# gk969/stm32-speech-recognition

Measured on AMD Instinct MI355X. Metric: utterances/sec (256-frame, 100 templates), higher is better.
Workload: dtype int32

## Files before the change

profiles/experiments/dtw_stats.py:

```python
import ctypes, json, os, sys
import numpy as np, torch
sys.path.insert(0, os.getcwd())
import bench
from stm32_speech_recognition_amd import Engine, synth
from stm32_speech_recognition_amd import engine as E

which = sys.argv[1] if len(sys.argv) > 1 else "ref"
gain = float(sys.argv[2]) if len(sys.argv) > 2 else 1.0
B = 8192
rate, cfg, Kt, n_words = bench.workload_setup(which, None)
dev = torch.device("cuda", 0)
bank = synth.word_bank(n_words)
eng = Engine(max_frames=bench.MAX_FRAMES, device=0, **cfg)
tm, tfr, rng = bench.make_templates(eng, bank, Kt, n_words, rate, dev, gain)
eng.set_templates_dense(tm, tfr.astype(np.uint32))
pcm = synth.make_utterances(torch.from_numpy(rng.integers(0, n_words, B)), [bench.T] * B, seed=1000, bank=bank,
                            S=synth.buf_len_for(bench.T, rate), device=dev, rate=rate, gain=gain)
out = eng.alloc_outputs(B, dev, mfcc=True, vad=True)
eng.set_pipeline(streams=1)
L = E.load_library()
st = (ctypes.c_ulonglong * 8)()
L.sr_debug_dtw_stats(st, 1)
eng.recognize_dev(pcm, out)
torch.cuda.synchronize()
L.sr_debug_dtw_stats(st, 1)
v = list(st)
sc = out["scores"].cpu().numpy().astype(np.int64)
print(json.dumps({"workload": which, "gain": gain, "wave_steps": v[0], "unsafe": v[1], "short": v[2], "beyond_table": v[3], "lost": v[4],
                  "lane_steps": v[5], "no_adv_y": v[6], "no_adv_x": v[7], "frac_no_adv_y": round(v[6] / v[0], 5),
                  "frac_no_adv_x": round(v[7] / v[0], 5), "frac_unsafe": round(v[1] / v[0], 5), "frac_short": round(v[2] / v[0], 5),
                  "frac_beyond": round(v[3] / v[0], 5), "frac_lost": round(v[4] / v[0], 5),
                  "score_median": float(np.median(sc[sc < 0xFFFFFFFF])), "score_p99": float(np.percentile(sc[sc < 0xFFFFFFFF], 99))}))
```

stm32_speech_recognition_amd/csrc/k_dtw.hip:

```cpp
#include "sr_dtw_dev.h"
#include "sr_dtw_plan.h"

namespace sr {

__device__ uint32_t dtw_pair(const int16_t *in, uint32_t in_n, uint32_t in_rows, const int16_t *mdl, uint32_t mdl_n,
                             uint32_t mdl_rows)
{
    if (in_n > mdl_n * 2 || 2 * in_n < mdl_n) return SR_DIS_ERR;
    const int X1 = (int)(((2 * (int)mdl_n - (int)in_n) / 3) & 0xFFFF);
    const int X2 = (int)(((4 * (int)in_n - 2 * (int)mdl_n) / 3) & 0xFFFF);
    uint32_t px = 0, py = 0;
    Frame12 ci = load_frame(in), cm = load_frame(mdl);
    uint32_t nci = norm2(ci), ncm = norm2(cm);
    uint32_t dis = get_dis_dev(ci, nci, cm, ncm);
    uint32_t step = 1;
    do {
        const uint32_t rx = (px + 1 < in_rows) ? px + 1 : in_rows - 1, ry = (py + 1 < mdl_rows) ? py + 1 : mdl_rows - 1;
        const Frame12 ni = load_frame(in + (size_t)rx * kCoef), nm = load_frame(mdl + (size_t)ry * kCoef);
        const uint32_t nni = norm2(ni), nnm = norm2(nm);
        const int x = (int)px + 1, y = (int)py + 1;
        const uint32_t up = dtw_out(x, y + 1, X1, X2, (int)in_n, (int)mdl_n) ? SR_DIS_ERR : get_dis_dev(nm, nnm, ci, nci);
        const uint32_t right = dtw_out(x + 1, y, X1, X2, (int)in_n, (int)mdl_n) ? SR_DIS_ERR : get_dis_dev(cm, ncm, ni, nni);
        const uint32_t diag =
            dtw_out(x + 1, y + 1, X1, X2, (int)in_n, (int)mdl_n) ? SR_DIS_ERR : get_dis_dev(nm, nnm, ni, nni);
// ... 344 lines not shown
                     "v_pk_mov_b32 %[c3], %[n3], %[n3] op_sel:[0,1]\n\t"
                     "v_pk_mov_b32 %[c4], %[n4], %[n4] op_sel:[0,1]\n\t"
                     "s_mov_b64 exec, %[live]"
                     : [c0] "+v"(c0), [c1] "+v"(c1), [c2] "+v"(c2), [c3] "+v"(c3), [c4] "+v"(c4)
                     : [n0] "v"(n0), [n1] "v"(n1), [n2] "v"(n2), [n3] "v"(n3), [n4] "v"(n4), [k_dg] "s"(k_dg), [k_up] "s"(k_up), [live] "s"(live)
                     : "scc");
        cm.w[0] = c0.x, cm.w[1] = c0.y, cm.w[2] = c1.x, cm.w[3] = c1.y, cm.w[4] = c2.x, cm.w[5] = c2.y, cm.w[6] = c3.x, cm.w[7] = c3.y;
        cm.w[8] = c4.x, cm.w[9] = c4.y;
        u32x4 q0 = {nm.w[0], nm.w[1], nm.w[2], nm.w[3]}, q1 = {nm.w[4], nm.w[5], nm.w[6], nm.w[7]};
        u32x2 q2 = {nm.w[8], nm.w[9]};
        u32x2 a0 = {ci.w[0], ci.w[1]}, a1 = {ci.w[2], ci.w[3]}, a2 = {ci.w[4], ci.w[5]}, a3 = {ci.w[6], ci.w[7]}, b0 = {ni.w[0], ni.w[1]},
              b1 = {ni.w[2], ni.w[3]}, b2 = {ni.w[4], ni.w[5]}, b3 = {ni.w[6], ni.w[7]}, an = {ci.w[8], ni.w[8]};
        asm volatile("s_or_b64 exec, %[k_dg], %[k_up]\n\t" SR_DTW_ADV_Y
                     "global_load_dwordx4 %[q0], %[t_off], %[tbase]\n\t"
                     "global_load_dwordx4 %[q1], %[t_off], %[tbase] offset:16\n\t"
                     "global_load_dwordx2 %[q2], %[t_off], %[tbase] offset:32\n\t" SR_DTW_ADV_X("32")
                     "ds_read_b64 %[a0], %[in_off]\n\t"
                     "ds_read_b64 %[a1], %[in_off] offset:8\n\t"
                     "ds_read_b64 %[a2], %[in_off] offset:16\n\t"
                     "ds_read_b64 %[a3], %[in_off] offset:24\n\t"
                     "ds_read_b64 %[b0], %[in_off] offset:32\n\t"
                     "ds_read_b64 %[b1], %[in_off] offset:40\n\t"
                     "ds_read_b64 %[b2], %[in_off] offset:48\n\t"
                     "ds_read_b64 %[b3], %[in_off] offset:56\n\t" SR_DTW_ADV_END
                     : [q0] "+v"(q0), [q1] "+v"(q1), [q2] "+v"(q2), [a0] "+v"(a0), [a1] "+v"(a1), [a2] "+v"(a2), [a3] "+v"(a3), [b0] "+v"(b0),
                       [b1] "+v"(b1), [b2] "+v"(b2), [b3] "+v"(b3), [an] "+v"(an), SR_DTW_ADV_OPS
                     : SR_DTW_ADV_INS
                     : "memory", "scc");
        nm.w[0] = q0.x, nm.w[1] = q0.y, nm.w[2] = q0.z, nm.w[3] = q0.w, nm.w[4] = q1.x, nm.w[5] = q1.y, nm.w[6] = q1.z, nm.w[7] = q1.w;
        nm.w[8] = q2.x, nm.w[9] = q2.y;
        ci.w[0] = a0.x, ci.w[1] = a0.y, ci.w[2] = a1.x, ci.w[3] = a1.y, ci.w[4] = a2.x, ci.w[5] = a2.y, ci.w[6] = a3.x, ci.w[7] = a3.y;
        ni.w[0] = b0.x, ni.w[1] = b0.y, ni.w[2] = b1.x, ni.w[3] = b1.y, ni.w[4] = b2.x, ni.w[5] = b2.y, ni.w[6] = b3.x, ni.w[7] = b3.y;
        ci.w[8] = an.x, ni.w[8] = an.y;
    }
    static __device__ __forceinline__ void wait_lds(Row &ci, Row &ni)
    {
        u32x2 a0 = {ci.w[0], ci.w[1]}, a1 = {ci.w[2], ci.w[3]}, a2 = {ci.w[4], ci.w[5]}, a3 = {ci.w[6], ci.w[7]}, b0 = {ni.w[0], ni.w[1]},
              b1 = {ni.w[2], ni.w[3]}, b2 = {ni.w[4], ni.w[5]}, b3 = {ni.w[6], ni.w[7]}, an = {ci.w[8], ni.w[8]};
        asm volatile("s_waitcnt lgkmcnt(0)" : "+v"(a0), "+v"(a1), "+v"(a2), "+v"(a3), "+v"(b0), "+v"(b1), "+v"(b2), "+v"(b3), "+v"(an));
        ci.w[0] = a0.x, ci.w[1] = a0.y, ci.w[2] = a1.x, ci.w[3] = a1.y, ci.w[4] = a2.x, ci.w[5] = a2.y, ci.w[6] = a3.x, ci.w[7] = a3.y;
        ni.w[0] = b0.x, ni.w[1] = b0.y, ni.w[2] = b1.x, ni.w[3] = b1.y, ni.w[4] = b2.x, ni.w[5] = b2.y, ni.w[6] = b3.x, ni.w[7] = b3.y;
        ci.w[8] = an.x, ni.w[8] = an.y;
    }
    static __device__ __forceinline__ void wait_tpl(Row &nm)
    {
        u32x4 q0 = {nm.w[0], nm.w[1], nm.w[2], nm.w[3]}, q1 = {nm.w[4], nm.w[5], nm.w[6], nm.w[7]};
        u32x2 q2 = {nm.w[8], nm.w[9]};
        asm volatile("s_waitcnt vmcnt(0)" : "+v"(q0), "+v"(q1), "+v"(q2));
        nm.w[0] = q0.x, nm.w[1] = q0.y, nm.w[2] = q0.z, nm.w[3] = q0.w, nm.w[4] = q1.x, nm.w[5] = q1.y, nm.w[6] = q1.z, nm.w[7] = q1.w;
        nm.w[8] = q2.x, nm.w[9] = q2.y;
    }
};
#ifdef SR_DTW_STATS
__device__ unsigned long long g_dtw_stats[8];
extern "C" void sr_debug_dtw_stats(unsigned long long *out, int reset)
{
    (void)hipDeviceSynchronize();
    (void)hipMemcpyFromSymbol(out, HIP_SYMBOL(g_dtw_stats), sizeof(g_dtw_stats));
    if (reset) {
        unsigned long long z[8] = {0};
        (void)hipMemcpyToSymbol(HIP_SYMBOL(g_dtw_stats), z, sizeof(z));
    }
}
#endif
template <class F>
__global__ void __launch_bounds__(1024) k_dtw_lds(const DtwLdsArgs a)
{
    typedef typename F::Row Row;
    extern __shared__ __attribute__((aligned(16))) u32x2 smem2[];
    const uint32_t U = a.U, R = a.d.max_frames, K = a.d.K;
    u32x2 *s_rows = smem2 + a.tie_g / 8;
    const uint32_t row_stride = dtw_lds_row_stride(R, F::kWords), nrm_stride = dtw_lds_nrm_stride(R);
    uint32_t *s_nrm = (uint32_t *)(s_rows + (size_t)U * (row_stride / 2));
    uint32_t *s_n = s_nrm + (size_t)U * nrm_stride + 8;
    const uint32_t tid = threadIdx.x, b0 = blockIdx.x * U;
    for (uint32_t i = tid; i < a.tie_g / 16; i += blockDim.x) ((u32x4 *)smem2)[i] = ((const u32x4 *)a.tie_delta)[i];

    if (tid < U) {
        const uint32_t b = b0 + tid;
        uint32_t n = 0;
        if (b < a.d.B) {
            if (a.d.in_frames) n = a.d.in_frames[b];
            else n = (a.d.vad[b].status == SR_ST_OK) ? a.d.vad[b].frm_num : 0u;
        }
        s_n[tid] = n;
    }
    __syncthreads();
    for (uint32_t u = 0; u < U; u++) {
        const uint32_t n = s_n[u];
        if (!n) continue;
        const uint32_t rows = (n + 1 < R) ? n + 1 : R;
        const uint32_t nc = a.d.n_coef;
        const uint2 *src = (const uint2 *)(a.d.mfcc + (size_t)(b0 + u) * R * kCoef);
        u32x2 *dst = s_rows + (size_t)u * (row_stride / 2);
        for (uint32_t r = tid; r < rows; r += blockDim.x) {
            uint32_t w[F::kWords];
            if (F::kWords == 6 && nc == (uint32_t)kCoef) {
                const uint2 q0 = src[3 * r], q1 = src[3 * r + 1], q2 = src[3 * r + 2];
                w[0] = q0.x, w[1] = q0.y, w[2] = q1.x, w[3] = q1.y, w[4] = q2.x, w[5] = q2.y;
            } else {
                const int16_t *p = a.d.mfcc + ((size_t)(b0 + u) * R + r) * nc;
#pragma unroll
                for (uint32_t i = 0; i < F::kWords; i++) {
                    const uint32_t lo = (2 * i < nc) ? (uint32_t)(uint16_t)p[2 * i] : 0u, hi = (2 * i + 1 < nc) ? (uint32_t)(uint16_t)p[2 * i + 1] : 0u;
                    w[i] = lo | (hi << 16);
                }
            }
            int nr = sdot2z(w[0], w[0]);
#pragma unroll
            for (uint32_t i = 1; i < F::kWords; i++) nr = sdot2(w[i], w[i], nr);
#pragma unroll
            for (uint32_t i = 0; i < F::kWords / 2; i++) dst[(F::kWords / 2) * r + i] = u32x2{w[2 * i], w[2 * i + 1]};
            s_nrm[u * nrm_stride + r] = (uint32_t)nr;
        }
    }
    __syncthreads();

    if (tid >= U * a.Kc) return;
    const uint32_t ks = blockIdx.y * a.Kc + tid / U, u = tid % U, b = b0 + u;
    if (b >= a.d.B || ks >= K) return;
    const uint32_t in_n = s_n[u], mdl_n = a.tpl_frames_s[ks];
    uint32_t score = SR_DIS_ERR;
    if (in_n && mdl_n && !(in_n > mdl_n * 2 || 2 * in_n < mdl_n)) {
        const int X1 = (int)(((2 * (int)mdl_n - (int)in_n) / 3) & 0xFFFF);
        const int X2 = (int)(((4 * (int)in_n - 2 * (int)mdl_n) / 3) & 0xFFFF);
        const int c1s = 3 - ((int)in_n - 2 * (int)mdl_n), c2s = ((int)mdl_n - 2 * (int)in_n) - 3;
        uint32_t in_off = lds_offset(s_rows + (size_t)u * (row_stride / 2));
        uint32_t nrm_off = lds_offset(s_nrm + (size_t)u * nrm_stride);
        const char *tbase = (const char *)a.tplR;
        uint32_t t_off = ks * F::kTplBytes;
        const uint32_t t_stride = K * F::kTplBytes;
        auto tpl_row = [&](uint32_t off) { return F::tpl_row(tbase + off); };
        Row cm = tpl_row(t_off);
        t_off += t_stride;
        Row nm = tpl_row(t_off);
        Row ci, ni;
        F::rows2(in_off, nrm_off, ci, ni);
        uint32_t dis = cvt_u32(sqrt_rn_int((float)(uint32_t)F::dot_acc(cm, ci, (int)(F::nrm(cm) + F::nrm(ci)))));
        const int c1s2 = c1s + 2;
        const uint32_t tie_g1 = a.tie_g - 1;
        auto ub1_of = [&](int xx) { return (xx < X1) ? 2 * xx + 2 : ((xx + c1s2) >> 1); };
        auto lb_of = [&](int xx) { return (xx < X2) ? (xx >> 1) : 2 * xx + c2s; };
        int xB = 2, y1 = 2;
        int ubA1 = ub1_of(1), lbB = lb_of(2), ubB1 = ub1_of(2);
        uint64_t lost = 0;
        uint32_t trips = 1, step = 1;
        const uint64_t entry = __builtin_amdgcn_ballot_w64(true);
        uint64_t live = entry, mc;
        do {
          do {
            F::wait_lds(ci, ni);
            const uint32_t d_rt = (uint32_t)F::dot_acc(cm, ni, (int)(F::nrm(cm) + F::nrm(ni)));
            __builtin_amdgcn_sched_barrier(0);
            F::wait_tpl(nm);
            const uint32_t d_up = (uint32_t)F::dot_acc(nm, ci, (int)(F::nrm(nm) + F::nrm(ci)));
            const uint32_t d_dg = (uint32_t)F::dot_acc(nm, ni, (int)(F::nrm(nm) + F::nrm(ni)));
            const uint64_t m_up = __builtin_amdgcn_ballot_w64(y1 < ubA1),
                           m_rt = __builtin_amdgcn_ballot_w64(lbB < y1),
                           m_dg = __builtin_amdgcn_ballot_w64(lbB <= y1) & __builtin_amdgcn_ballot_w64(y1 < ubB1);
            uint32_t m2;
            asm volatile("v_cndmask_b32_e64 %0, -1, %5, %2\n\t"
                         "s_and_b64 exec, %1, %3\n\t"
                         "v_min_u32 %0, %0, %6\n\t"
                         "s_and_b64 exec, %1, %4\n\t"
                         "v_min_u32 %0, %0, %7\n\t"
                         "s_mov_b64 exec, %1"
                         : "=&v"(m2)
                         : "s"(live), "s"(m_dg), "s"(m_rt), "s"(m_up), "v"(d_dg), "v"(d_rt), "v"(d_up)
                         : "scc");
            uint32_t mn = sqrt_floor_low(m2);
            uint32_t T;
            {
                const int dl = *(lds_c_i8 *)(uintptr_t)mn;
                const uint32_t mp2 = mn + 2;
                asm("v_mad_u32_u24 %0, %1, %2, %3" : "=v"(T) : "v"(mn), "v"(mp2), "v"(dl));
            }
            uint64_t k_dg = m_dg & __builtin_amdgcn_ballot_w64(d_dg < T);
            uint64_t k_up = m_up & __builtin_amdgcn_ballot_w64(d_up < T) & ~k_dg;
            const uint64_t rare = __builtin_amdgcn_ballot_w64(m2 >= T) | __builtin_amdgcn_ballot_w64(mn >= tie_g1) | lost;
#ifdef SR_DTW_STATS
            {
                const uint64_t mb = __builtin_amdgcn_ballot_w64(m2 >= T), mr = __builtin_amdgcn_ballot_w64(mn >= tie_g1);
                if (__builtin_amdgcn_mbcnt_hi(~0u, __builtin_amdgcn_mbcnt_lo(~0u, 0)) == 0) {
                    atomicAdd(&g_dtw_stats[0], 1ull);
                    atomicAdd(&g_dtw_stats[5], (unsigned long long)__builtin_popcountll(live));
                    if (rare) atomicAdd(&g_dtw_stats[1], 1ull);
                    if (mb) atomicAdd(&g_dtw_stats[2], 1ull);
                    if (mr) atomicAdd(&g_dtw_stats[3], 1ull);
                    if (lost) atomicAdd(&g_dtw_stats[4], 1ull);
                }
            }
#endif
            if (__builtin_expect(rare != 0ull, 0)) {
                if (((__builtin_amdgcn_ballot_w64(mn >= tie_g1) | lost) == 0ull)) {
                    const uint32_t inc = (m2 >= T) ? 1u : 0u;
                    asm volatile("v_add_u32 %0, %1, %0" : "+v"(mn) : "v"(inc));
                    const int dl = *(lds_c_i8 *)(uintptr_t)mn;
                    const uint32_t T2 = mn * (mn + 2) + (uint32_t)dl;
                    k_dg = m_dg & __builtin_amdgcn_ballot_w64(d_dg < T2);
                    k_up = m_up & __builtin_amdgcn_ballot_w64(d_up < T2) & ~k_dg;
                } else {
                    const int x = xB - 1, y = y1 - 1;
                    const bool in_up = !dtw_out(x, y1, X1, X2, (int)in_n, (int)mdl_n), in_rt = !dtw_out(xB, y, X1, X2, (int)in_n, (int)mdl_n),
                               in_dg = !dtw_out(xB, y1, X1, X2, (int)in_n, (int)mdl_n);
                    const uint32_t up = in_up ? cvt_u32(sqrt_rn_int((float)d_up)) : SR_DIS_ERR,
                                   right = in_rt ? cvt_u32(sqrt_rn_int((float)d_rt)) : SR_DIS_ERR,
                                   diag = in_dg ? cvt_u32(sqrt_rn_int((float)d_dg)) : SR_DIS_ERR;
                    uint32_t mnl = diag;
                    if (mnl > right) mnl = right;
                    if (mnl > up) mnl = up;
                    asm volatile("v_mov_b32 %0, %1" : "+v"(mn) : "v"(mnl));
                    k_dg = __builtin_amdgcn_ballot_w64(mnl == diag);
                    k_up = __builtin_amdgcn_ballot_w64(mnl == up) & ~k_dg;
                    lost |= __builtin_amdgcn_ballot_w64(!(in_up | in_rt | in_dg));
                }
            }
#ifdef SR_DTW_STATS
            if (__builtin_amdgcn_mbcnt_hi(~0u, __builtin_amdgcn_mbcnt_lo(~0u, 0)) == 0) {
                if (!(k_dg | k_up)) atomicAdd(&g_dtw_stats[6], 1ull);
                if (!(live & ~k_up)) atomicAdd(&g_dtw_stats[7], 1ull);
            }
#endif
            asm volatile("v_add_u32 %0, %1, %0" : "+v"(dis) : "v"(mn));
            F::advance(cm, nm, ci, ni, tbase, t_off, t_stride, y1, in_off, nrm_off, xB, ubA1, ubB1, k_dg, k_up, live);
            {
                int ua, lb;
                asm("v_lshl_add_u32 %0, %1, 1, 2" : "=v"(ua) : "v"(xB));
                asm("v_lshl_add_u32 %0, %1, 1, %2" : "=v"(lb) : "v"(xB), "v"(c2s));
                const int ub = (xB + c1s2) >> 1, la = xB >> 1;
                const uint64_t m1 = __builtin_amdgcn_ballot_w64(xB < X1), m2x = __builtin_amdgcn_ballot_w64(xB < X2);
                asm volatile("s_nop 1\n\tv_cndmask_b32_e64 %0, %1, %2, %3" : "+v"(ubB1) : "v"(ub), "v"(ua), "s"(m1));
                asm volatile("v_cndmask_b32_e64 %0, %1, %2, %3" : "+v"(lbB) : "v"(lb), "v"(la), "s"(m2x));
            }
            trips++;
            mc = __builtin_amdgcn_ballot_w64(xB <= (int)in_n) & __builtin_amdgcn_ballot_w64(y1 <= (int)mdl_n);
          } while (__builtin_expect(mc == live, 1));
          asm volatile("s_andn2_b64 exec, %2, %3\n\t"
                       "v_mov_b32 %0, %1\n\t"
                       "s_mov_b64 exec, %3"
                       : "+v"(step)
                       : "s"(trips), "s"(live), "s"(mc)
                       : "scc");
          lost &= mc;
          live = mc;
        } while (live != 0ull);
        asm volatile("s_waitcnt vmcnt(0) lgkmcnt(0)\n\ts_mov_b64 exec, %2" : "+v"(dis), "+v"(step) : "s"(entry) : "memory");
        score = dis / step;
    }
    a.d.scores[(size_t)b * K + a.tpl_orig[ks]] = score;
}

__host__ __device__ inline size_t dtw_lds_fixed(uint32_t U, uint32_t max_frames, uint32_t row_words = 6)
{
    const size_t per_u = (size_t)(dtw_lds_row_stride(max_frames, row_words) + dtw_lds_nrm_stride(max_frames)) * 4;
    return U * per_u + 32 + ((4 * (size_t)U + 15) & ~(size_t)15);
}
uint32_t dtw_lds_pick_u(uint32_t K, uint32_t max_frames, const LdsBudget &budget, uint32_t *lds_bytes, uint32_t *tie_g,
                        uint32_t *kc_out, uint32_t row_words)
{
    const uint32_t kMinTie = 4096;
    uint32_t best_u = 0, best_g = 0, best_kc = 0;
    double best = 0;
    const uint32_t force = (uint32_t)dev_hook(kHookDtwU), force_g = (uint32_t)dev_hook(kHookDtwTieG),
                   force_kc = (uint32_t)dev_hook(kHookDtwKc);
    for (uint32_t U = 1; U <= (uint32_t)kDtwMaxU; U++) {
        uint32_t kc = K < 1024u / U ? K : 1024u / U;
        if (force_kc >= 1 && force_kc < kc) kc = force_kc;
        if (!kc) break;
        const uint32_t chunks = (K + kc - 1) / kc;
        if (chunks > 65535) continue;
        kc = (K + chunks - 1) / chunks;
        const uint64_t pairs = (uint64_t)U * kc;
        const size_t lds = dtw_lds_fixed(U, max_frames, row_words);
        if (lds + kMinTie > budget.stage_cap) break;
        const uint32_t waves = (uint32_t)((pairs + 63) / 64);
        uint32_t blocks = budget.wgs_per_cu(lds + kMinTie);
        if (blocks > 32 / waves) blocks = 32 / waves;
        if (blocks > 8) blocks = 8;
        if (blocks < 1) continue;
        uint32_t g = kMinTie;
        while (g < (uint32_t)kTieMax && budget.wgs_per_cu(lds + 2 * g) >= blocks) g *= 2;
        if (force_g >= kMinTie && force_g <= (uint32_t)kTieMax) {
            g = force_g & ~1023u;
            if (budget.wgs_per_cu(lds + g) < 1) continue;
        }
        const double eff = (double)K / ((double)chunks * 64.0 * waves / U);
        const double resident = (double)(blocks * waves);
        const double w = 0.5 * (K >= 400 ? 1.0 : K / 400.0);
        const double cover = g >= 16384 ? 1.0 : g >= 8192 ? 0.98 : 0.9;
        const double share = (1.0 - w / U) * (1.0 - 0.005 * (chunks - 1)) * cover;
        double score = eff * (resident >= 24 ? 1.0 : resident / 24.0) * share;
        if (force && force == U) score = 100.0;
        if (score > best + 1e-9) {
            best = score;
            best_u = U;
            best_g = g;
            best_kc = kc;
        }
    }
    if (best_u && lds_bytes) *lds_bytes = (uint32_t)(dtw_lds_fixed(best_u, max_frames, row_words) + best_g);
// ... 79 lines not shown
```

stm32_speech_recognition_amd/csrc/k_misc.hip:

```cpp
#include "sr_dtw_dev.h"
#ifdef SR_TESTING
#include <algorithm>
#include <cstdio>
#include <mutex>
#include <string>
#include <vector>
#endif

namespace sr {

__global__ void __launch_bounds__(256) k_delta_mfcc(const int16_t *mfcc, const sr_vad_rec *vad, const uint32_t *frames,
                                                    uint32_t B, uint32_t max_frames, uint32_t nc, int16_t *delta)
{
    const uint64_t i = (uint64_t)blockIdx.x * blockDim.x + threadIdx.x;
    const uint32_t per = max_frames * nc;
    if (i >= (uint64_t)B * per) return;
    const uint32_t b = (uint32_t)(i / per), r = (uint32_t)(i - (uint64_t)b * per), t = r / nc, c = r - t * nc;
    uint32_t n = frames ? frames[b] : ((vad[b].status == SR_ST_OK) ? vad[b].frm_num : 0u);
    if (n > max_frames) n = max_frames;
    int16_t out = 0;
    if (t < n) {
        const int16_t *m = mfcc + (uint64_t)b * per + c;
        const uint32_t p1 = t + 1 < n ? t + 1 : n - 1, p2 = t + 2 < n ? t + 2 : n - 1;
        const uint32_t m1 = t >= 1 ? t - 1 : 0, m2 = t >= 2 ? t - 2 : 0;
        const int num = ((int)m[p1 * nc] - (int)m[m1 * nc]) + 2 * ((int)m[p2 * nc] - (int)m[m2 * nc]);
        out = (int16_t)(num / 10);
    }
    delta[i] = out;
}
void launch_delta_mfcc(const int16_t *mfcc, const sr_vad_rec *vad, const uint32_t *frames, uint32_t B, uint32_t max_frames,
                       uint32_t n_coef, int16_t *delta, hipStream_t s)
{
    const uint64_t n = (uint64_t)B * max_frames * n_coef;
    if (!n) return;
    SR_LAUNCH_POINT(s, "k_delta_mfcc");
    hipLaunchKernelGGL(k_delta_mfcc, dim3((uint32_t)((n + 255) / 256)), dim3(256), 0, s, mfcc, vad, frames, B, max_frames, n_coef, delta);
}

__global__ void __launch_bounds__(256) k_unpack12(const uint32_t *packed, uint64_t row_words, uint16_t *out, uint64_t out_stride,
                                                  uint32_t groups_per_row, uint32_t B)
{
    const uint64_t i = (uint64_t)blockIdx.x * blockDim.x + threadIdx.x;
    if (i >= (uint64_t)B * groups_per_row) return;
    const uint32_t b = (uint32_t)(i / groups_per_row), g = (uint32_t)(i - (uint64_t)b * groups_per_row);
    const uint32_t *src = packed + (uint64_t)b * row_words + 3ull * g;
    const uint32_t w0 = src[0], w1 = src[1], w2 = src[2];
    const uint32_t s0 = w0 & 0xFFFu, s1 = (w0 >> 12) & 0xFFFu, s2 = (w0 >> 24) | ((w1 & 0xFu) << 8), s3 = (w1 >> 4) & 0xFFFu;
    const uint32_t s4 = (w1 >> 16) & 0xFFFu, s5 = (w1 >> 28) | ((w2 & 0xFFu) << 4), s6 = (w2 >> 8) & 0xFFFu, s7 = w2 >> 20;
    *(uint4 *)(out + (uint64_t)b * out_stride + 8ull * g) = make_uint4(s0 | s1 << 16, s2 | s3 << 16, s4 | s5 << 16, s6 | s7 << 16);
}
void launch_unpack12(const void *packed, uint64_t row_bytes, uint16_t *out, uint64_t out_stride, uint32_t buf_len, uint32_t B,
                     hipStream_t s)
{
    const uint32_t groups = (buf_len + 7) / 8;
    const uint64_t n = (uint64_t)B * groups;
    if (!n) return;
    SR_LAUNCH_POINT(s, "k_unpack12");
    hipLaunchKernelGGL(k_unpack12, dim3((uint32_t)((n + 255) / 256)), dim3(256), 0, s, (const uint32_t *)packed, row_bytes / 4, out,
                       out_stride, groups, B);
}

__global__ void k_math_diag(const uint32_t *in, uint32_t *out, uint32_t n, const uint32_t *log_thr)
{
    const uint32_t i = blockIdx.x * blockDim.x + threadIdx.x;
    if (i >= n) return;
    const uint32_t x = in[i];
    out[3 * i + 0] = log100_u32(x, log_thr);
    {
        const uint32_t q = sqrt_floor_low(x), e = cvt_u32(sqrt_rn_int((float)x));
        out[3 * i + 1] = (q == e || q + 1 == e) ? e : 0xDEAD0001u;
    }
    out[3 * i + 2] = cvt_u32(sqrt_rn_int((float)(int)(x & 0x7FFFFFFFu)) * 10.0f);
}
void launch_math_diag(const uint32_t *in, uint32_t *out, uint32_t n, const DevTables &t, hipStream_t s)
{
    if (!n) return;
    SR_LAUNCH_POINT(s, "k_math_diag");
    hipLaunchKernelGGL(k_math_diag, dim3((n + 255) / 256), dim3(256), 0, s, in, out, n, t.log_thr);
}

__global__ void __launch_bounds__(256) k_mel_term_sweep(uint32_t tri_lo, uint32_t e_max, unsigned long long *bad)
{
    const uint32_t tri = tri_lo + blockIdx.y, m = mel_fused_multiplier(tri);
    unsigned long long n = 0;
    if (mel_tri_of_multiplier(m) != tri) n += 1ull << 40;
    for (uint64_t e = (uint64_t)blockIdx.x * blockDim.x + threadIdx.x; e <= e_max; e += (uint64_t)gridDim.x * blockDim.x) {
        const uint32_t E = (uint32_t)e;
        const uint32_t ref = E * tri / 100u;
        n += (mel_term_fused(E << 4, m) != ref) || ((uint64_t)E * tri / 100u != ref);
    }
    if (n) atomicAdd(bad + blockIdx.y, n);
}
__global__ void __launch_bounds__(256) k_mag_fast_sweep(uint32_t n_max, unsigned long long *bad, uint32_t *first_bad)
{
    unsigned long long c = 0;
    for (uint64_t i = (uint64_t)blockIdx.x * blockDim.x + threadIdx.x; i <= (n_max & 0x7FFFFFFFu); i += (uint64_t)gridDim.x * blockDim.x) {
        const uint32_t n = (uint32_t)i;
        uint32_t want, got;
        if (n_max & 0x80000000u) {
            want = cvt_u32(sqrt_rn_int((float)n));
            got = cvt_u32(__builtin_amdgcn_sqrtf((float)n));
        } else {
            want = cvt_u32(sqrt_rn_int((float)(int)n) * 10.0f);
            got = mag10_small((float)(int)n);
        }
        if (want != got) {
            c++;
            atomicMin(first_bad, n);
        }
    }
    if (c) atomicAdd(bad, c);
}
void launch_mag_fast_sweep(uint32_t n_max, unsigned long long *bad, uint32_t *first_bad, hipStream_t s)
{
    SR_LAUNCH_POINT(s, "k_mag_fast_sweep");
    hipLaunchKernelGGL(k_mag_fast_sweep, dim3(1024), dim3(256), 0, s, n_max, bad, first_bad);
}
void launch_mel_term_sweep(uint32_t tri_lo, uint32_t n_tri, uint32_t e_max, unsigned long long *bad, hipStream_t s)
{
    if (!n_tri) return;
    SR_LAUNCH_POINT(s, "k_mel_term_sweep");
    hipLaunchKernelGGL(k_mel_term_sweep, dim3(256, n_tri), dim3(256), 0, s, tri_lo, e_max, bad);
}

__global__ void k_get_dis(const int16_t *pa, const int16_t *pb, uint32_t *out, uint32_t n)
{
    const uint32_t i = blockIdx.x * blockDim.x + threadIdx.x;
    if (i >= n) return;
    const Frame12 fa = load_frame(pa + (size_t)i * kCoef), fb = load_frame(pb + (size_t)i * kCoef);
    out[i] = get_dis_dev(fa, norm2(fa), fb, norm2(fb));
}
// ... 126 lines not shown
```

stm32_speech_recognition_amd/csrc/sr_device.h:

```cpp
#pragma once
#include <hip/hip_runtime.h>

#include <cstdint>

#include "../../include/sr_engine.h"
#include "sr_onepass_plan.h"

namespace sr {

enum DevHook {
    kHookDtwU,
    kHookDtwTieG,
    kHookDtwKc,
    kHookMfccGrid,
    kHookPerturbLogThr,
    kHookLogThrFromHost,
    kHookMultiAllowDup,
    kHookDtwDebug,
    kHookCellsLiteral,
    kHookMagCheapOff,
    kHookMagTableOff,
    kHookStreamTile,
    kHookSpotChunk,
    kHookAlignPairs,
    kHookAlignGlobal,
    kHookChainChunk,
    kHookChainRows,
    kHookSpanGroups,
    kHookClusterPairs,
    kHookForcedPruneOff,
    kHookOnePassBlock,
    kHookOnePassRows,
    kHookOnePassGramPruneOff,
    kHookLiveOrigin,
    kHookSpotLiveOrigin,
    kHookLdsPoisonLaunches,
    kHookCount
};
#ifdef SR_TESTING
int64_t dev_hook(DevHook h);
#else
constexpr int64_t dev_hook(DevHook) { return 0; }
#endif

constexpr uint32_t kPoisonHigh = 0, kPoisonLow = 1;
#ifdef SR_TESTING
void launch_point(hipStream_t s, const char *kernel);
void launch_points_reset();
uint64_t launch_points_seen(char *names, size_t names_cap);
int launch_lds_probe(uint32_t words, uint32_t *d_out, hipStream_t s);
#define SR_LAUNCH_POINT(stream, name) ::sr::launch_point((stream), (name))
#else
#define SR_LAUNCH_POINT(stream, name) ((void)0)
#endif

struct DevTables {
    const uint16_t *hamm;
    const uint16_t *tri_even;
    const uint16_t *tri_odd;
    const uint16_t *tri_cen;
    const int8_t *dct;
    const uint32_t *tw_a;
    const uint32_t *tw_b;
    const uint32_t *log_thr;
    const uint32_t *tri_even32;
    const uint32_t *tri_odd32;
    const uint32_t *tri_even_m;
    const uint32_t *tri_odd_m;
    const uint32_t *w512_a;
    const uint32_t *w512_b;
    const int8_t *tie_delta;
    const uint32_t *hamm_pk;
};

struct VadArgs {
    const uint16_t *pcm;
    uint64_t pcm_stride;
    uint32_t buf_len;
    uint32_t noise_len;
    uint32_t atap_frm;
    uint32_t max_frames;
    uint32_t max_seg;
    uint32_t B;
    sr_vad_rec *vad;
    const sr_atap *atap_in;
    uint64_t *dbg_masks;
    uint32_t frame_len;
    uint32_t v_durmin;
    uint32_t s_durmax;
// ... 609 lines not shown
```

stm32_speech_recognition_amd/csrc/sr_dtw_dev.h:

```cpp
#pragma once
#include "sr_dev.h"

namespace sr {

struct Frame12 {
    uint32_t w[6];
};
__device__ __forceinline__ Frame12 load_frame(const int16_t *p)
{
    const uint2 *q = (const uint2 *)p;
    const uint2 a = q[0], b = q[1], c = q[2];
    Frame12 f;
    f.w[0] = a.x;
    f.w[1] = a.y;
    f.w[2] = b.x;
    f.w[3] = b.y;
    f.w[4] = c.x;
    f.w[5] = c.y;
    return f;
}
__device__ __forceinline__ uint32_t norm2(const Frame12 &f)
{
    int acc = 0;
#pragma unroll
    for (int i = 0; i < 6; i++) acc = sdot2(f.w[i], f.w[i], acc);
    return (uint32_t)acc;
}
__device__ __forceinline__ uint32_t get_dis_dev(const Frame12 &fa, uint32_t na, const Frame12 &fb, uint32_t nb)
{
    int dot = 0;
#pragma unroll
    for (int i = 0; i < 6; i++) dot = sdot2(fa.w[i], fb.w[i], dot);
    const uint32_t d = na + nb - 2u * (uint32_t)dot;
    return cvt_u32(sqrt_rn_int((float)d));
}
__device__ __forceinline__ bool dtw_out(int x, int y, int X1, int X2, int in_n, int mdl_n)
{
    const bool o1 = (x < X1) ? (y >= 2 * x + 2) : (2 * y + in_n - 2 * mdl_n >= x + 4);
    const bool o2 = (x < X2) ? (2 * y + 2 <= x) : (y + 4 <= 2 * x + mdl_n - 2 * in_n);
    return o1 || o2;
}

__device__ __forceinline__ uint32_t dis_from(uint32_t na, uint32_t nb, int dot)
{
    const uint32_t d = na + nb - 2u * (uint32_t)dot;
    return cvt_u32(sqrt_rn_int((float)d));
}

__device__ __forceinline__ uint32_t sqrt_floor_low(uint32_t d)
{
    const float s0 = __builtin_amdgcn_sqrtf((float)d);
    uint32_t r;
    asm("v_cvt_u32_f32 %0, %1" : "=v"(r) : "v"(__int_as_float(__float_as_int(s0) - 1)));
    return r;
}
__device__ __forceinline__ uint32_t sub_sat(uint32_t a, uint32_t b)
{
    uint32_t r;
    asm("v_sub_u32_e64 %0, %1, %2 clamp" : "=v"(r) : "v"(a), "v"(b));
    return r;
}

struct Row32 {
    uint32_t w[8];
};
__device__ __forceinline__ Row32 row_from(const u32x4 lo, const u32x4 hi)
{
    Row32 r;
    r.w[0] = lo.x; r.w[1] = lo.y; r.w[2] = lo.z; r.w[3] = lo.w;
    r.w[4] = hi.x; r.w[5] = hi.y; r.w[6] = hi.z; r.w[7] = hi.w;
    return r;
}
__device__ __forceinline__ Row32 row_from2(const u32x2 a, const u32x2 b, const u32x2 c, uint32_t nrm)
{
    Row32 r;
    r.w[0] = a.x; r.w[1] = a.y; r.w[2] = b.x; r.w[3] = b.y; r.w[4] = c.x; r.w[5] = c.y;
    r.w[6] = nrm; r.w[7] = 0;
    return r;
}
__device__ __forceinline__ void copy_row(Row32 &dst, const Row32 &src)
{
#pragma unroll
    for (int i = 0; i < 8; i += 2) {
        u32x2 d;
        const u32x2 v = {src.w[i], src.w[i + 1]};
        asm("v_pk_mov_b32 %0, %1, %1 op_sel:[0,1]" : "=v"(d) : "v"(v));
        dst.w[i] = d.x;
        dst.w[i + 1] = d.y;
    }
}
__device__ __forceinline__ int dot_rows(const Row32 &a, const Row32 &b)
{
    int acc = sdot2z(a.w[0], b.w[0]);
#pragma unroll
    for (int i = 1; i < 6; i++) acc = sdot2(a.w[i], b.w[i], acc);
    return acc;
}

__device__ __forceinline__ int dot_rows_acc(const Row32 &a, const Row32 &b, int c)
{
    int acc = sdot2a(a.w[0], b.w[0], c);
#pragma unroll
    for (int i = 1; i < 6; i++) acc = sdot2(a.w[i], b.w[i], acc);
    return acc;
}

}
```

stm32_speech_recognition_amd/csrc/sr_engine.cpp:

```cpp
#include "sr_engine_internal.h"

#include <atomic>
#include <cstdio>
#include <cstdlib>

namespace sr {

static thread_local std::string g_err;
int set_error(int code, const std::string &msg)
{
    g_err = msg;
    return code;
}

#ifdef SR_TESTING
static std::atomic<int64_t> g_hooks[kHookCount];
int64_t dev_hook(DevHook h) { return g_hooks[h].load(std::memory_order_relaxed); }
static const char *const kHookNames[kHookCount] = {"dtw_u", "dtw_tie_g", "dtw_kc", "mfcc_grid", "perturb_log_thr",
                                                   "log_thr_from_host", "multi_allow_dup", "dtw_debug", "cells_literal",
                                                   "mag_cheap_off", "mag_table_off", "stream_tile_frames", "spot_chunk_cols",
                                                   "align_pairs", "align_marks_global", "chain_chunk_cols", "chain_rows", "span_groups",
                                                   "cluster_pairs", "forced_prune_off", "onepass_block", "onepass_rows", "onepass_gram_prune_off", "live_origin",
                                                   "spot_live_origin", "lds_poison_launches"};
#endif
}

using namespace sr;

static int check_device(int want, int *out_dev)
{
    int n = 0;
    hipError_t e = hipGetDeviceCount(&n);
    if (e != hipSuccess || n <= 0)
        return fail(SR_ERR_NO_DEVICE, std::string("no HIP device: ") + (e != hipSuccess ? hipGetErrorString(e) : "count 0"));
    int dev = want;
    if (dev < 0) {
        if (hipGetDevice(&dev) != hipSuccess) dev = 0;
    }
    if (dev >= n) return fail(SR_ERR_NO_DEVICE, "device ordinal out of range");
    hipDeviceProp_t prop;
    if (hipGetDeviceProperties(&prop, dev) != hipSuccess) return fail(SR_ERR_NO_DEVICE, "hipGetDeviceProperties failed");
    if (std::strncmp(prop.gcnArchName, "gfx950", 6) != 0)
        return fail(SR_ERR_NO_DEVICE, std::string("kernels are built for gfx950 only, device is ") + prop.gcnArchName);
    *out_dev = dev;
    return SR_OK;
}

extern "C" {

const char *sr_last_error(void) { return g_err.c_str(); }

void sr_default_config(sr_config *c)
{
    c->fs = 8000;
    c->frame_time_ms = 20;
    c->frame_mov_ms = 10;
    c->nfft = 1024;
    c->n_mel = 24;
    c->n_coef = 12;
    c->max_frames = 119;
    c->noise_len_ms = 300;
    c->max_seg = 3;
    c->device = -1;
}

static int front_end_of(const sr_config *cfg, FrontEnd *fe)
{
    const bool is_ref = cfg->fs == 8000 && cfg->nfft == 1024 && cfg->n_mel == 24;
    const bool is_ext = cfg->fs == 16000 && cfg->nfft == 512 && cfg->n_mel == 40;
    if ((is_ref || is_ext) && cfg->frame_time_ms == 20 && cfg->frame_mov_ms == 10 && cfg->n_coef == 12) {
        *fe = is_ext ? kFrontExt : kFrontRef;
        return SR_OK;
    }
    const char *what = "supported: fs=8000/nfft=1024/24 Mel/12 MFCC (reference), fs=16000/nfft=512/40 Mel/12 MFCC (extension), or the generic "
                       "front end: nfft=1024, fs a multiple of 4000, frame_time_ms = 2*frame_mov_ms with frame_len in {160,240,256,320,400,512}, "
                       "n_mel even 4..64, n_coef 1..16";
// ... 592 lines not shown
```

stm32_speech_recognition_amd/csrc/sr_tables.cpp:

```cpp
#include "sr_device.h"
#include "sr_tables.h"

#include <atomic>
#include <cmath>
#include <cstdio>
#include <cstdlib>

namespace sr {

static const uint32_t kLogThrRef[kLogMax + 2] = {
#include "sr_log_thr_ref.inc"
};
static std::atomic<int> g_log_mismatches{0};
int log_table_mismatches() { return g_log_mismatches.load(); }

static double mround(double v) { return v >= 0.0 ? std::floor(v + 0.5) : -std::floor(-v + 0.5); }

static void gen_hamm(HostTables &t, const FrontEnd &fe)
{
    t.hamm.resize(fe.frame_len);
    for (int i = 0; i < fe.frame_len; i++)
        t.hamm[i] = (uint16_t)mround((0.54 - 0.46 * std::cos(2 * M_PI * i / (fe.frame_len - 1))) * 10000.0);
}

// ... 71 lines not shown
    for (int N = 16; N <= kNfft; N *= 4)
        for (int b = 0; b < N / 4; b++)
            for (int e = 0; e < 3; e++, n++) {
                double th = 2.0 * M_PI * (mult[e] * b) / N;
                int kr = (int)mround(16384.0 * (std::cos(th) - std::sin(th)));
                int ki = (int)mround(16384.0 * std::sin(th));
                int kc = kr + ki, ks = ki;
                t.tw_kr[n] = (int16_t)kr;
                t.tw_ki[n] = (int16_t)ki;
                t.tw_a[n] = ((uint32_t)kc & 0xFFFFu) | ((uint32_t)ks << 16);
                t.tw_b[n] = ((uint32_t)(-ks) & 0xFFFFu) | ((uint32_t)kc << 16);
            }
}

static uint32_t log100(uint32_t n) { return n ? (uint32_t)(std::log((double)n) * 100) : 0u; }

static void gen_log_thr(HostTables &t)
{
    t.log_thr.assign(kLogMax + 2, 0xFFFFFFFFu);
    t.log_thr[0] = 1;
    for (int m = 1; m <= kLogMax; m++) {
        uint64_t lo = t.log_thr[m - 1], hi = 0xFFFFFFFFull;
        while (lo < hi) {
            uint64_t mid = (lo + hi) / 2;
            if (log100((uint32_t)mid) >= (uint32_t)m)
                hi = mid;
            else
                lo = mid + 1;
        }
        t.log_thr[m] = (uint32_t)lo;
    }
    {
        const int64_t m = dev_hook(kHookPerturbLogThr);
        if (m >= 1 && m <= kLogMax) t.log_thr[m] += 1;
    }
    const bool keep = dev_hook(kHookLogThrFromHost) != 0;
    int bad = 0;
    for (int m = 0; m <= kLogMax + 1; m++) bad += t.log_thr[m] != kLogThrRef[m];
    g_log_mismatches.store(bad);
    if (bad && !keep) t.log_thr.assign(kLogThrRef, kLogThrRef + kLogMax + 2);
}

static uint32_t root_u32(uint32_t d) { return (uint32_t)sqrtf((float)d); }

static void gen_tie_delta(HostTables &t)
{
    t.tie_delta.assign(kTieMax, 1);
    for (uint32_t g = 4095; g < (uint32_t)kTieMax; g++) {
        const uint64_t M = (uint64_t)(g + 1) * (g + 1);
        uint32_t d = (uint32_t)M;
        while (root_u32(d - 1) >= g + 1) d--;
        const int64_t delta = (int64_t)d - (int64_t)M + 1;
        t.tie_delta[g] = (int8_t)delta;
        if (delta < -128 || delta > 127) t.tie_delta.clear();
    }
}

void gen_mag_q(std::vector<uint16_t> &out)
{
    out.resize(kMagTabEntries);
    for (uint32_t n = 0; n < kMagTabEntries; n++) out[n] = (uint16_t)(((uint32_t)(sqrtf((float)n) * 10.0f)) << 2);
}

void build_tables(HostTables &t, const FrontEnd &fe)
{
    gen_mag_q(t.mag_q);
    gen_tie_delta(t);
    gen_hamm(t, fe);
    gen_tri(t, fe);
    gen_dct(t, fe);
    gen_twiddles(t);
    gen_log_thr(t);
    gen_w512(t);
}

}
```

stm32_speech_recognition_amd/csrc/sr_tables.h:

```cpp
#pragma once
#include <cstdint>
#include <vector>

namespace sr {

constexpr int kFrameLen = 160;
constexpr int kHop = 80;
constexpr int kNfft = 1024;
constexpr int kBins = 512;
constexpr int kMel = 24;
constexpr int kCoef = 12;
constexpr int kTwiddles = 1020;
constexpr int kLogMax = 2218;
constexpr int kTieMax = 32768;


constexpr int kWinShift = 5;
constexpr int32_t hamm_fused_multiplier(uint32_t h) { return (int32_t)((((uint64_t)h << 27) + 999u) / 1000u); }

constexpr uint32_t kMelFusedMaxE = (1u << 28) / 100u;
constexpr uint32_t kMagSmallMax = 26843;
static_assert(1638u * 1638u <= kMelFusedMaxE && 100ull * (kMagSmallMax + 1) < 1639ull * 1639ull, "quiet-frame bound");
constexpr uint32_t kMagCheapMax = 70171;
static_assert(kMagSmallMax <= kMagCheapMax, "the quiet tier lies inside the cheap-magnitude range");
constexpr uint32_t kMagTabEntries = kMagSmallMax + 1;
static_assert((1638u << 2) <= 0xFFFFu && 2 * kMagTabEntries < (1u << 17), "table entries fit u16, table fits a raw buffer's range");
constexpr uint32_t kMelTriMax = 1599;
constexpr uint32_t mel_fused_multiplier(uint32_t tri) { return (uint32_t)((((uint64_t)tri << 28) + 99u) / 100u); }

struct FrontEnd {
    int fs, frame_len, hop, nfft, bins, n_mel, n_coef;
    bool generic;
};
constexpr FrontEnd kFrontRef = {8000, 160, 80, 1024, 512, 24, 12, false};
constexpr FrontEnd kFrontExt = {16000, 320, 160, 512, 256, 40, 12, false};

struct HostTables {
    std::vector<uint16_t> hamm;
    std::vector<uint16_t> tri_cen;
    std::vector<uint16_t> tri_even;
    std::vector<uint16_t> tri_odd;
    std::vector<int8_t> dct;
    std::vector<uint32_t> tw_a, tw_b;
    std::vector<int16_t> tw_kr, tw_ki;
    std::vector<uint32_t> log_thr;
    std::vector<uint32_t> w512_a, w512_b;
    std::vector<int8_t> tie_delta;
    std::vector<uint16_t> mag_q;
};

void build_tables(HostTables &t, const FrontEnd &fe);
void gen_mag_q(std::vector<uint16_t> &out);
int log_table_mismatches();

}
```

Before: 3.553 million.

## Run unchecked DTW trip batches when all lanes are far from bounds; use ceil-root tie table

The DTW wavefront loop is split into a lambda trip and an outer scheduler. When every live lane has at least a minimum slack before its sequence ends, the wave computes the minimum slack with a DPP reduction and runs that many trips without the per-trip exit ballot. The rounding step switches from a floor square root plus a (mn+2) multiply to a ceil square root with a pre-shifted tie-delta table built in LDS, which saves an add per trip. The final score is corrected by subtracting step-1. This adds diagnostic and stats paths, and risks subtle rounding or exit-condition errors.

```diff
diff --git a/profiles/experiments/dtw_stats.py b/profiles/experiments/dtw_stats.py
--- a/profiles/experiments/dtw_stats.py
+++ b/profiles/experiments/dtw_stats.py
@@ -19,7 +19,7 @@
 out = eng.alloc_outputs(B, dev, mfcc=True, vad=True)
 eng.set_pipeline(streams=1)
 L = E.load_library()
-st = (ctypes.c_ulonglong * 8)()
+st = (ctypes.c_ulonglong * 12)()
 L.sr_debug_dtw_stats(st, 1)
 eng.recognize_dev(pcm, out)
 torch.cuda.synchronize()
@@ -30,4 +30,6 @@
                   "lane_steps": v[5], "no_adv_y": v[6], "no_adv_x": v[7], "frac_no_adv_y": round(v[6] / v[0], 5),
                   "frac_no_adv_x": round(v[7] / v[0], 5), "frac_unsafe": round(v[1] / v[0], 5), "frac_short": round(v[2] / v[0], 5),
                   "frac_beyond": round(v[3] / v[0], 5), "frac_lost": round(v[4] / v[0], 5),
+                  "trips_untested": v[8], "trips_tested": v[9], "budgets": v[10], "budget_gates": v[11],
+                  "frac_untested": round(v[8] / max(v[8] + v[9], 1), 5), "trips_per_budget": round(v[8] / max(v[10], 1), 2),
                   "score_median": float(np.median(sc[sc < 0xFFFFFFFF])), "score_p99": float(np.percentile(sc[sc < 0xFFFFFFFF], 99))}))
diff --git a/stm32_speech_recognition_amd/csrc/k_dtw.hip b/stm32_speech_recognition_amd/csrc/k_dtw.hip
--- a/stm32_speech_recognition_amd/csrc/k_dtw.hip
+++ b/stm32_speech_recognition_amd/csrc/k_dtw.hip
@@ -420,17 +420,25 @@
     }
 };
 #ifdef SR_DTW_STATS
-__device__ unsigned long long g_dtw_stats[8];
+__device__ unsigned long long g_dtw_stats[12];
 extern "C" void sr_debug_dtw_stats(unsigned long long *out, int reset)
 {
     (void)hipDeviceSynchronize();
     (void)hipMemcpyFromSymbol(out, HIP_SYMBOL(g_dtw_stats), sizeof(g_dtw_stats));
     if (reset) {
-        unsigned long long z[8] = {0};
+        unsigned long long z[12] = {0};
         (void)hipMemcpyToSymbol(HIP_SYMBOL(g_dtw_stats), z, sizeof(z));
     }
 }
+#define SR_DTW_STAT_ADD(i, v)                                                                                           \
+    do {                                                                                                                \
+        if (__builtin_amdgcn_mbcnt_hi((uint32_t)(live >> 32), __builtin_amdgcn_mbcnt_lo((uint32_t)live, 0)) == 0)       \
+            atomicAdd(&g_dtw_stats[i], v);                                                                              \
+    } while (0)
+#else
+#define SR_DTW_STAT_ADD(i, v) ((void)0)
 #endif
+constexpr uint32_t kDtwMinRun = 16;
 template <class F>
 __global__ void __launch_bounds__(1024) k_dtw_lds(const DtwLdsArgs a)
 {
@@ -442,7 +450,11 @@
     uint32_t *s_nrm = (uint32_t *)(s_rows + (size_t)U * (row_stride / 2));
     uint32_t *s_n = s_nrm + (size_t)U * nrm_stride + 8;
     const uint32_t tid = threadIdx.x, b0 = blockIdx.x * U;
-    for (uint32_t i = tid; i < a.tie_g / 16; i += blockDim.x) ((u32x4 *)smem2)[i] = ((const u32x4 *)a.tie_delta)[i];
+    for (uint32_t i = tid; i < a.tie_g / 16; i += blockDim.x) {
+        const u32x4 q = ((const u32x4 *)a.tie_delta)[i];
+        const uint32_t below = i ? ((const uint32_t *)a.tie_delta)[4 * i - 1] : kTieBelowFirst;
+        ((u32x4 *)smem2)[i] = u32x4{dtw_t1_word(q.x, below), dtw_t1_word(q.y, q.x), dtw_t1_word(q.z, q.y), dtw_t1_word(q.w, q.z)};
+    }
 
     if (tid < U) {
         const uint32_t b = b0 + tid;
@@ -514,9 +526,8 @@
         uint64_t lost = 0;
         uint32_t trips = 1, step = 1;
         const uint64_t entry = __builtin_amdgcn_ballot_w64(true);
-        uint64_t live = entry, mc;
-        do {
-          do {
+        uint64_t live = entry, mc, near = 0;
+        auto trip = [&]() __attribute__((always_inline)) {
             F::wait_lds(ci, ni);
             const uint32_t d_rt = (uint32_t)F::dot_acc(cm, ni, (int)(F::nrm(cm) + F::nrm(ni)));
             __builtin_amdgcn_sched_barrier(0);
@@ -536,19 +547,18 @@
                          : "=&v"(m2)
                          : "s"(live), "s"(m_dg), "s"(m_rt), "s"(m_up), "v"(d_dg), "v"(d_rt), "v"(d_up)
                          : "scc");
-            uint32_t mn = sqrt_floor_low(m2);
+            uint32_t r1 = sqrt_ceil_low(m2);
             uint32_t T;
             {
-                const int dl = *(lds_c_i8 *)(uintptr_t)mn;
-                const uint32_t mp2 = mn + 2;
-                asm("v_mad_u32_u24 %0, %1, %2, %3" : "=v"(T) : "v"(mn), "v"(mp2), "v"(dl));
+                const int dl = *(lds_c_i8 *)(uintptr_t)r1;
+                asm("v_mad_u32_u24 %0, %1, %1, %2" : "=v"(T) : "v"(r1), "v"(dl));
             }
             uint64_t k_dg = m_dg & __builtin_amdgcn_ballot_w64(d_dg < T);
             uint64_t k_up = m_up & __builtin_amdgcn_ballot_w64(d_up < T) & ~k_dg;
-            const uint64_t rare = __builtin_amdgcn_ballot_w64(m2 >= T) | __builtin_amdgcn_ballot_w64(mn >= tie_g1) | lost;
+            const uint64_t rare = __builtin_amdgcn_ballot_w64(m2 >= T) | __builtin_amdgcn_ballot_w64(r1 >= tie_g1) | lost;
 #ifdef SR_DTW_STATS
             {
-                const uint64_t mb = __builtin_amdgcn_ballot_w64(m2 >= T), mr = __builtin_amdgcn_ballot_w64(mn >= tie_g1);
+                const uint64_t mb = __builtin_amdgcn_ballot_w64(m2 >= T), mr = __builtin_amdgcn_ballot_w64(r1 >= tie_g1);
                 if (__builtin_amdgcn_mbcnt_hi(~0u, __builtin_amdgcn_mbcnt_lo(~0u, 0)) == 0) {
                     atomicAdd(&g_dtw_stats[0], 1ull);
                     atomicAdd(&g_dtw_stats[5], (unsigned long long)__builtin_popcountll(live));
@@ -560,11 +570,11 @@
             }
 #endif
             if (__builtin_expect(rare != 0ull, 0)) {
-                if (((__builtin_amdgcn_ballot_w64(mn >= tie_g1) | lost) == 0ull)) {
+                if (((__builtin_amdgcn_ballot_w64(r1 >= tie_g1) | lost) == 0ull)) {
                     const uint32_t inc = (m2 >= T) ? 1u : 0u;
-                    asm volatile("v_add_u32 %0, %1, %0" : "+v"(mn) : "v"(inc));
-                    const int dl = *(lds_c_i8 *)(uintptr_t)mn;
-                    const uint32_t T2 = mn * (mn + 2) + (uint32_t)dl;
+                    asm volatile("v_add_u32 %0, %1, %0" : "+v"(r1) : "v"(inc));
+                    const int dl = *(lds_c_i8 *)(uintptr_t)r1;
+                    const uint32_t T2 = r1 * r1 + (uint32_t)dl;
                     k_dg = m_dg & __builtin_amdgcn_ballot_w64(d_dg < T2);
                     k_up = m_up & __builtin_amdgcn_ballot_w64(d_up < T2) & ~k_dg;
                 } else {
@@ -577,7 +587,7 @@
                     uint32_t mnl = diag;
                     if (mnl > right) mnl = right;
                     if (mnl > up) mnl = up;
-                    asm volatile("v_mov_b32 %0, %1" : "+v"(mn) : "v"(mnl));
+                    asm volatile("v_add_u32 %0, 1, %1" : "+v"(r1) : "v"(mnl));
                     k_dg = __builtin_amdgcn_ballot_w64(mnl == diag);
                     k_up = __builtin_amdgcn_ballot_w64(mnl == up) & ~k_dg;
                     lost |= __builtin_amdgcn_ballot_w64(!(in_up | in_rt | in_dg));
@@ -589,7 +599,7 @@
                 if (!(live & ~k_up)) atomicAdd(&g_dtw_stats[7], 1ull);
             }
 #endif
-            asm volatile("v_add_u32 %0, %1, %0" : "+v"(dis) : "v"(mn));
+            asm volatile("v_add_u32 %0, %1, %0" : "+v"(dis) : "v"(r1));
             F::advance(cm, nm, ci, ni, tbase, t_off, t_stride, y1, in_off, nrm_off, xB, ubA1, ubB1, k_dg, k_up, live);
             {
                 int ua, lb;
@@ -600,6 +610,23 @@
                 asm volatile("s_nop 1\n\tv_cndmask_b32_e64 %0, %1, %2, %3" : "+v"(ubB1) : "v"(ub), "v"(ua), "s"(m1));
                 asm volatile("v_cndmask_b32_e64 %0, %1, %2, %3" : "+v"(lbB) : "v"(lb), "v"(la), "s"(m2x));
             }
+        };
+        do {
+          while ((near & live) == 0ull) {
+              const int slack = min((int)in_n - xB, (int)mdl_n - y1);
+              SR_DTW_STAT_ADD(11, 1ull);
+              near = live & ~__builtin_amdgcn_ballot_w64(slack >= (int)kDtwMinRun);
+              if (near) break;
+              uint32_t run = wave_min_live(slack, live);
+              SR_DTW_STAT_ADD(10, 1ull);
+              SR_DTW_STAT_ADD(8, (unsigned long long)run);
+              trips += run;
+              do trip();
+              while (--run);
+          }
+          do {
+            trip();
+            SR_DTW_STAT_ADD(9, 1ull);
             trips++;
             mc = __builtin_amdgcn_ballot_w64(xB <= (int)in_n) & __builtin_amdgcn_ballot_w64(y1 <= (int)mdl_n);
           } while (__builtin_expect(mc == live, 1));
@@ -613,7 +640,7 @@
           live = mc;
         } while (live != 0ull);
         asm volatile("s_waitcnt vmcnt(0) lgkmcnt(0)\n\ts_mov_b64 exec, %2" : "+v"(dis), "+v"(step) : "s"(entry) : "memory");
-        score = dis / step;
+        score = (dis - (step - 1)) / step;
     }
     a.d.scores[(size_t)b * K + a.tpl_orig[ks]] = score;
 }
diff --git a/stm32_speech_recognition_amd/csrc/k_misc.hip b/stm32_speech_recognition_amd/csrc/k_misc.hip
--- a/stm32_speech_recognition_amd/csrc/k_misc.hip
+++ b/stm32_speech_recognition_amd/csrc/k_misc.hip
@@ -60,15 +60,46 @@
                        out_stride, groups, B);
 }
 
-__global__ void k_math_diag(const uint32_t *in, uint32_t *out, uint32_t n, const uint32_t *log_thr)
+__device__ __forceinline__ uint32_t root1_poison(uint32_t d, uint32_t e, const int8_t *tie_delta)
+{
+    const uint32_t r1 = sqrt_ceil_low(d), q = sqrt_floor_low(d);
+    if (!(r1 == e + 1 || r1 == e)) return 0xDEAD0002u;
+    if (r1 < (uint32_t)kTieMax) {
+        const uint32_t T = r1 * r1 + (uint32_t)(r1 ? (int)tie_delta[r1 - 1] - 1 : 0);
+        if ((d >= T) != (r1 == e)) return 0xDEAD0003u;
+    }
+    if (!(q == e || q + 1 == e)) return 0xDEAD0001u;
+    return 0;
+}
+__global__ void k_math_diag(const uint32_t *in, uint32_t *out, uint32_t n, const uint32_t *log_thr, const int8_t *tie_delta, uint32_t mode)
 {
     const uint32_t i = blockIdx.x * blockDim.x + threadIdx.x;
     if (i >= n) return;
     const uint32_t x = in[i];
+    if (mode == 2) {
+        const uint32_t d0 = x << 12;
+        uint32_t prev = d0 ? cvt_u32(sqrt_rn_int((float)(d0 - 1))) : 0u, bad = 0, shorts = 0;
+        for (uint32_t j = 0; j < 4096; j++) {
+            const uint32_t d = d0 + j, e = cvt_u32(sqrt_rn_int((float)d));
+            uint32_t p = root1_poison(d, e, tie_delta);
+            if (e < prev) p = 0xDEAD0004u;
+            if (!bad) bad = p;
+            shorts += sqrt_ceil_low(d) == e ? 1u : 0u;
+            prev = e;
+        }
+        out[3 * i + 0] = shorts;
+        out[3 * i + 1] = bad;
+        out[3 * i + 2] = prev;
+        return;
+    }
     out[3 * i + 0] = log100_u32(x, log_thr);
     {
         const uint32_t q = sqrt_floor_low(x), e = cvt_u32(sqrt_rn_int((float)x));
         out[3 * i + 1] = (q == e || q + 1 == e) ? e : 0xDEAD0001u;
+        if (mode == 1) {
+            const uint32_t p = root1_poison(x, e, tie_delta);
+            if (p) out[3 * i + 1] = p;
+        }
     }
     out[3 * i + 2] = cvt_u32(sqrt_rn_int((float)(int)(x & 0x7FFFFFFFu)) * 10.0f);
 }
@@ -76,7 +107,8 @@
 {
     if (!n) return;
     SR_LAUNCH_POINT(s, "k_math_diag");
-    hipLaunchKernelGGL(k_math_diag, dim3((n + 255) / 256), dim3(256), 0, s, in, out, n, t.log_thr);
+    hipLaunchKernelGGL(k_math_diag, dim3((n + 255) / 256), dim3(256), 0, s, in, out, n, t.log_thr, t.tie_delta,
+                       (uint32_t)dev_hook(kHookMathDiagRoot1));
 }
 
 __global__ void __launch_bounds__(256) k_mel_term_sweep(uint32_t tri_lo, uint32_t e_max, unsigned long long *bad)
diff --git a/stm32_speech_recognition_amd/csrc/sr_device.h b/stm32_speech_recognition_amd/csrc/sr_device.h
--- a/stm32_speech_recognition_amd/csrc/sr_device.h
+++ b/stm32_speech_recognition_amd/csrc/sr_device.h
@@ -35,6 +35,7 @@
     kHookLiveOrigin,
     kHookSpotLiveOrigin,
     kHookLdsPoisonLaunches,
+    kHookMathDiagRoot1,
     kHookCount
 };
 #ifdef SR_TESTING
diff --git a/stm32_speech_recognition_amd/csrc/sr_dtw_dev.h b/stm32_speech_recognition_amd/csrc/sr_dtw_dev.h
--- a/stm32_speech_recognition_amd/csrc/sr_dtw_dev.h
+++ b/stm32_speech_recognition_amd/csrc/sr_dtw_dev.h
@@ -54,6 +54,38 @@
     asm("v_cvt_u32_f32 %0, %1" : "=v"(r) : "v"(__int_as_float(__float_as_int(s0) - 1)));
     return r;
 }
+__device__ __forceinline__ uint32_t sqrt_ceil_low(uint32_t d)
+{
+    const float s0 = __builtin_amdgcn_sqrtf((float)d);
+    uint32_t r;
+    asm("v_cvt_u32_f32 %0, %1" : "=v"(r) : "v"(__builtin_ceilf(s0)));
+    return r;
+}
+__device__ __forceinline__ uint32_t wave_min_live(int v, uint64_t live)
+{
+    uint32_t t, r;
+    asm volatile("s_mov_b64 exec, -1\n\t"
+                 "v_cndmask_b32_e64 %[t], -1, %[v], %[live]\n\t"
+                 "s_nop 1\n\t"
+                 "v_min_u32_dpp %[t], %[t], %[t] row_ror:1 row_mask:0xf bank_mask:0xf\n\t"
+                 "s_nop 1\n\t"
+                 "v_min_u32_dpp %[t], %[t], %[t] row_ror:2 row_mask:0xf bank_mask:0xf\n\t"
+                 "s_nop 1\n\t"
+                 "v_min_u32_dpp %[t], %[t], %[t] row_ror:4 row_mask:0xf bank_mask:0xf\n\t"
+                 "s_nop 1\n\t"
+                 "v_min_u32_dpp %[t], %[t], %[t] row_ror:8 row_mask:0xf bank_mask:0xf\n\t"
+                 "s_nop 1\n\t"
+                 "v_min_u32_dpp %[t], %[t], %[t] row_bcast:15 row_mask:0xa bank_mask:0xf\n\t"
+                 "s_nop 1\n\t"
+                 "v_min_u32_dpp %[t], %[t], %[t] row_bcast:31 row_mask:0xc bank_mask:0xf\n\t"
+                 "s_nop 1\n\t"
+                 "v_readlane_b32 %[r], %[t], 63\n\t"
+                 "s_mov_b64 exec, %[live]"
+                 : [t] "=&v"(t), [r] "=&s"(r)
+                 : [v] "v"(v), [live] "s"(live)
+                 : "scc");
+    return r;
+}
 __device__ __forceinline__ uint32_t sub_sat(uint32_t a, uint32_t b)
 {
     uint32_t r;
diff --git a/stm32_speech_recognition_amd/csrc/sr_engine.cpp b/stm32_speech_recognition_amd/csrc/sr_engine.cpp
--- a/stm32_speech_recognition_amd/csrc/sr_engine.cpp
+++ b/stm32_speech_recognition_amd/csrc/sr_engine.cpp
@@ -21,7 +21,7 @@
                                                    "mag_cheap_off", "mag_table_off", "stream_tile_frames", "spot_chunk_cols",
                                                    "align_pairs", "align_marks_global", "chain_chunk_cols", "chain_rows", "span_groups",
                                                    "cluster_pairs", "forced_prune_off", "onepass_block", "onepass_rows", "onepass_gram_prune_off", "live_origin",
-                                                   "spot_live_origin", "lds_poison_launches"};
+                                                   "spot_live_origin", "lds_poison_launches", "math_diag_root1"};
 #endif
 }
 
diff --git a/stm32_speech_recognition_amd/csrc/sr_tables.cpp b/stm32_speech_recognition_amd/csrc/sr_tables.cpp
--- a/stm32_speech_recognition_amd/csrc/sr_tables.cpp
+++ b/stm32_speech_recognition_amd/csrc/sr_tables.cpp
@@ -147,7 +147,10 @@
         while (root_u32(d - 1) >= g + 1) d--;
         const int64_t delta = (int64_t)d - (int64_t)M + 1;
         t.tie_delta[g] = (int8_t)delta;
-        if (delta < -128 || delta > 127) t.tie_delta.clear();
+        if (delta < kTieDeltaMin || delta > kTieDeltaMax) {
+            t.tie_delta.clear();
+            return;
+        }
     }
 }
 
diff --git a/stm32_speech_recognition_amd/csrc/sr_tables.h b/stm32_speech_recognition_amd/csrc/sr_tables.h
--- a/stm32_speech_recognition_amd/csrc/sr_tables.h
+++ b/stm32_speech_recognition_amd/csrc/sr_tables.h
@@ -13,6 +13,12 @@
 constexpr int kTwiddles = 1020;
 constexpr int kLogMax = 2218;
 constexpr int kTieMax = 32768;
+constexpr int kTieDeltaMin = -127, kTieDeltaMax = 127;
+constexpr uint32_t kTieBelowFirst = 0x01000000u;
+constexpr uint32_t dtw_t1_word(uint32_t w, uint32_t below)
+{
+    return ((((w << 8) | (below >> 24)) ^ 0x80808080u) - 0x01010101u) ^ 0x80808080u;
+}
 
 
 constexpr int kWinShift = 5;
```

After: 3.552 million. Within noise of the previous version (-0.0%).
